# mindazhao/PWStableNet

Hardware: AMD Instinct MI355X
Metric: stabilized frames/sec at 256x256 (netG fp32 + grid_sample), whole job (higher is better)
Workload: dtype f32

## Files before the change

### pwstablenet_amd/csrc/conv_dispatch.hip

```cpp
#include "conv_common.h"

namespace pws {

static inline bool ledger_direct(int bit) { return (exp_mask(EXP_PARITY_LEDGER, 32) & bit) != 0; }

int conv2d_fwd_impl(const pws_conv_args *a, const ConvCtx &cx) {
    PWS_REQUIRE(a != nullptr, "pws_conv2d_fwd: args is NULL");
    PWS_REQUIRE(a->n >= 0 && a->h > 0 && a->w > 0, "pws_conv2d_fwd: bad n/h/w %d/%d/%d", a->n, a->h, a->w);
    PWS_REQUIRE(a->nsrc >= 1 && a->nsrc <= 4, "pws_conv2d_fwd: nsrc %d not in 1..4", a->nsrc);
    PWS_REQUIRE(a->cout > 0 && a->cout % 4 == 0, "pws_conv2d_fwd: cout %d must be a positive multiple of 4", a->cout);
    PWS_REQUIRE(a->out && a->w_packed, "pws_conv2d_fwd: NULL out / w_packed");
    PWS_REQUIRE(a->out_ld >= a->cout, "pws_conv2d_fwd: out_ld %d < cout %d", a->out_ld, a->cout);
    PWS_REQUIRE(a->act >= PWS_ACT_NONE && a->act <= PWS_ACT_RELU, "pws_conv2d_fwd: bad act %d", a->act);
    PWS_REQUIRE(a->ws == nullptr || (reinterpret_cast<size_t>(a->ws) & 15) == 0, "pws_conv2d_fwd: ws must be 16-B aligned");
    if (a->n == 0) return PWS_OK;

    ConvKParams kp{};
    int cin = 0;
    kp.nsrc = a->nsrc;
    const bool nchw = a->src_nchw != 0;
    if (nchw) {
        PWS_REQUIRE(a->kind == PWS_CONV_K5S1 && a->nsrc == 1, "pws_conv2d_fwd: NCHW source only for the k5 first layer");
        PWS_REQUIRE(a->src[0].ptr && a->src[0].channels > 0, "pws_conv2d_fwd: bad NCHW source");
        PWS_REQUIRE(a->src[0].ld >= 0, "pws_conv2d_fwd: NCHW source: ld is the sample stride in floats (0 = dense)");
        kp.src_ptr[0] = a->src[0].ptr, kp.src_c[0] = a->src[0].channels, kp.src_ld[0] = a->src[0].ld;
        cin = a->src[0].channels;
    } else {
        for (int s = 0; s < a->nsrc; ++s) {
            const pws_src &sr = a->src[s];
            PWS_REQUIRE(sr.ptr && sr.channels > 0 && sr.channels % 16 == 0 && sr.ld >= sr.channels && sr.ld % 4 == 0 &&
                            (reinterpret_cast<size_t>(sr.ptr) & 15) == 0,
                        "pws_conv2d_fwd: source %d (channels %d, ld %d) must be 16-B aligned, channels %% 16 == 0, ld %% 4 == 0",
                        s, sr.channels, sr.ld);
            kp.src_ptr[s] = sr.ptr, kp.src_c[s] = sr.channels, kp.src_ld[s] = sr.ld;
            cin += sr.channels;
        }
    }
    kp.cin_pad = (cin + 15) / 16 * 16;
    kp.N = a->n, kp.H = a->h, kp.W = a->w;
    kp.cout = a->cout, kp.w = a->w_packed, kp.bias = a->bias, kp.out_ld = a->out_ld, kp.act = a->act;
    kp.nclasses = 1;
    PWS_REQUIRE((size_t)a->n * a->h * a->w < (1u << 31), "pws_conv2d_fwd: n*h*w too large for 32-bit pixel indices");
    float *ws = static_cast<float *>(a->ws);
    const size_t ws_floats = a->ws_bytes / sizeof(float);
    const bool bf16 = a->math == PWS_MATH_BF16 && a->w_bf16 && !nchw;
    if (a->store == PWS_STORE_BF16) {
        PWS_REQUIRE(bf16, "pws_conv2d_fwd: bf16 storage needs math == PWS_MATH_BF16, w_bf16 and NHWC sources");
        PWS_REQUIRE(a->out_ld % 2 == 0 && a->cout % 2 == 0 && (reinterpret_cast<size_t>(a->out) & 3) == 0,
                    "pws_conv2d_fwd: bf16 storage needs an even cout / out_ld and a 4-byte aligned out");
        for (int s = 0; s < a->nsrc; ++s)
            PWS_REQUIRE(a->src[s].channels % 32 == 0 && a->src[s].ld % 8 == 0,
                        "pws_conv2d_fwd: bf16 storage needs channels %% 32 == 0 and ld %% 8 == 0 (source %d: %d, %d)", s,
                        a->src[s].channels, a->src[s].ld);
        kp.io_bf16 = 1;
        kp.epi16 = a->cout % 8 == 0 && a->out_ld % 8 == 0 && (reinterpret_cast<size_t>(a->out) & 15) == 0;
    }
    kp.w_bf = a->w_bf16, kp.kpad_bf = (kp.cin_pad + 31) / 32 * 32, kp.npad_bf = (a->cout + 63) / 64 * 64;
    if (a->out_sign) {
        PWS_REQUIRE(a->store == PWS_STORE_BF16 && a->cout % 8 == 0 && a->out_sign_ld >= a->cout / 8,
                    "pws_conv2d_fwd: out_sign needs bf16 storage, cout %% 8 == 0 and out_sign_ld >= cout / 8");
        kp.out_sign = a->out_sign, kp.out_sign_ld = a->out_sign_ld;
    }

    const bool fp32_nhwc = !bf16 && !nchw, k5 = a->kind == PWS_CONV_K5S1;
    const bool ringf_on = fp32_nhwc && !k5 && !ledger_direct(8), skinny_on = fp32_nhwc && !k5 && !ledger_direct(16);
    int k2;
    bool wring_on = false, wino_on = false;
    switch (a->kind) {
    case PWS_CONV_K3S1:
    case PWS_CONVT_K3S1: {
        kp.OH = kp.LH = a->h, kp.OW = kp.LW = a->w, k2 = 9;
        wring_on = a->w_wring && fp32_nhwc && !ledger_direct(2);
        const long wblocks = cdiv(a->w, 16) * cdiv(a->h, 16) * a->n * cdiv(a->cout, 64);
        wino_on = a->w_wino && !nchw && a->h >= 16 && a->w >= 16 && wblocks >= 128 && (cin >= 128 || wblocks >= 2048) && !ledger_direct(2);
        break;
    }
    case PWS_CONV_K3S2: kp.OH = kp.LH = (a->h + 2 - 3) / 2 + 1, kp.OW = kp.LW = (a->w + 2 - 3) / 2 + 1, k2 = 9; break;
    case PWS_CONV_K5S1:
        kp.OH = kp.LH = a->h, kp.OW = kp.LW = a->w, k2 = 25;
        ws = nullptr;
        break;
    case PWS_CONVT_K4S2: {
        kp.LH = a->h, kp.LW = a->w, kp.OH = 2 * a->h, kp.OW = 2 * a->w, kp.nclasses = 4, k2 = 4;
        wring_on = a->w_wring && fp32_nhwc && !ledger_direct(4);
        const long wb = cdiv(a->w, 24) * cdiv(a->h, 12) * a->n * cdiv(a->cout, 64) * 4;
        wino_on = a->w_wino && a->h >= 24 && a->w >= 24 && wb >= 256 && !ledger_direct(4);
        break;
    }
    default:
        set_error("pws_conv2d_fwd: kind %d is not a runnable conv kind", a->kind);
        return PWS_EINVAL;
    }
    const double out_pix = (double)a->n * kp.OH * kp.OW, es = a->store == PWS_STORE_BF16 ? 2.0 : 4.0, ws_ = bf16 ? 2.0 : 4.0;
    ProfInfo pi{2.0 * out_pix * a->cout * (double)cin * k2, es * ((double)a->n * a->h * a->w * cin + out_pix * a->cout) + ws_ * (double)k2 * cin * a->cout};
    if (a->kind == PWS_CONVT_K4S2) pi.bytes += ws_ * 12.0 * cin * a->cout;
    int rc = PWS_OK;
    if (bf16 && conv_bf16_fwd(a->kind, kp, kp.cin_pad, a->out, ws, ws_floats, pi, cx, &rc)) return rc;
    if (wring_on && conv_wring(a, pi, cx, &rc)) return rc;
    if (wino_on && conv_wino(a, pi, cx, &rc)) return rc;
    kp.out = a->out;
    if (ringf_on && conv_ringf(a->kind, kp, pi, cx, &rc)) return rc;
    if (skinny_on && conv_skinny(a->kind, kp, a->out, ws, ws_floats, pi, cx, &rc)) return rc;
    if (k5 && nchw && !ledger_direct(1)) {
        if (a->w_wring && conv_first_wino(kp, static_cast<const float *>(a->w_wring), pi, cx, &rc)) return rc;
        if (conv_first(kp, pi, cx, &rc)) return rc;
    }
    conv_mfma(a->kind, false, nchw, kp, kp.cin_pad, a->out, ws, ws_floats, pi, cx, &rc);
    return rc;
}

int conv2d_bwd_data_impl(const pws_conv_bwd_data_args *a, const ConvCtx &cx) {
    PWS_REQUIRE(a != nullptr, "pws_conv2d_bwd_data: args is NULL");
    PWS_REQUIRE(a->n >= 0 && a->h > 0 && a->w > 0 && a->cout > 0 && a->cout % 16 == 0, "pws_conv2d_bwd_data: bad shape");
    PWS_REQUIRE(a->gout && a->w_dgrad && a->gout_ld >= a->cout && a->gout_ld % 4 == 0, "pws_conv2d_bwd_data: bad gout / weights");
    PWS_REQUIRE(a->ndst >= 1 && a->ndst <= 4, "pws_conv2d_bwd_data: ndst %d not in 1..4", a->ndst);
    if (a->n == 0) return PWS_OK;
    ConvKParams kp{};
    int oh = a->h, ow = a->w;
    if (a->kind == PWS_CONV_K3S2) oh = (a->h - 1) / 2 + 1, ow = (a->w - 1) / 2 + 1;
    if (a->kind == PWS_CONVT_K4S2) oh = 2 * a->h, ow = 2 * a->w;
    kp.nsrc = 1, kp.src_ptr[0] = a->gout, kp.src_c[0] = a->cout, kp.src_ld[0] = a->gout_ld;
    kp.N = a->n, kp.H = oh, kp.W = ow;
    kp.OH = a->h, kp.OW = a->w;
    kp.cin_pad = a->cout;
    int cin_f = 0;
    kp.ndst = a->ndst;
    for (int s = 0; s < a->ndst; ++s) {
        const pws_dst &d = a->dst[s];
        PWS_REQUIRE(d.ptr && d.channels > 0 && d.ld >= d.channels, "pws_conv2d_bwd_data: bad destination %d", s);
        kp.dst_ptr[s] = d.ptr, kp.dst_c0[s] = cin_f, kp.dst_c1[s] = cin_f + d.channels, kp.dst_ld[s] = d.ld;
        kp.dst_acc[s] = d.accumulate ? 1 : 0;
        if (d.act_y && d.act != PWS_ACT_NONE) {
            PWS_REQUIRE(a->store == PWS_STORE_BF16 && (d.act == PWS_ACT_LRELU || d.act == PWS_ACT_RELU),
                        "pws_conv2d_bwd_data: the fused act' (dst[%d].act_y) needs bf16 storage and PWS_ACT_LRELU / PWS_ACT_RELU", s);
            PWS_REQUIRE(d.act_y_ld >= d.channels && d.act_y_ld % 2 == 0 && (reinterpret_cast<size_t>(d.act_y) & 3) == 0,
                        "pws_conv2d_bwd_data: bad act_y / act_y_ld of destination %d", s);
            kp.dst_y[s] = d.act_y, kp.dst_y_ld[s] = d.act_y_ld, kp.dst_act[s] = d.act;
            if (d.act_sign) {
                PWS_REQUIRE(d.channels % 8 == 0 && d.act_sign_ld >= d.channels / 8, "pws_conv2d_bwd_data: bad act_sign / act_sign_ld of destination %d", s);
                kp.dst_sign[s] = d.act_sign, kp.dst_sign_ld[s] = d.act_sign_ld;
            }
        }
        cin_f += d.channels;
    }
    PWS_REQUIRE(cin_f % 4 == 0, "pws_conv2d_bwd_data: total destination channels %d must be a multiple of 4", cin_f);
    kp.cout = cin_f, kp.w = a->w_dgrad, kp.bias = nullptr, kp.act = PWS_ACT_NONE, kp.out_ld = cin_f, kp.nclasses = 1;
    PWS_REQUIRE((size_t)a->n * oh * ow < (1u << 31) && (size_t)a->n * a->h * a->w < (1u << 31), "pws_conv2d_bwd_data: too large");
    float *ws = static_cast<float *>(a->ws);
    const size_t ws_floats = a->ws_bytes / sizeof(float);
    ProfInfo pi;
    const double k2 = a->kind == PWS_CONVT_K4S2 ? 4.0 : 9.0;
    pi.flops = 2.0 * a->n * oh * ow * (double)a->cout * cin_f * k2;
    {
        const double es = a->store == PWS_STORE_BF16 ? 2.0 : 4.0, in_pix = (double)a->n * a->h * a->w;
        pi.bytes = es * ((double)a->n * oh * ow * a->cout + in_pix * cin_f);
        for (int s = 0; s < a->ndst; ++s)
            pi.bytes += es * in_pix * a->dst[s].channels * (a->dst[s].accumulate ? 1.0 : 0.0) +
                        (kp.dst_act[s] == PWS_ACT_NONE ? 0.0 : (kp.dst_sign[s] ? in_pix * a->dst[s].channels / 8.0 : es * in_pix * a->dst[s].channels));
    }
    if (a->kind == PWS_CONV_K3S2)
        kp.LH = oh, kp.LW = ow, kp.nclasses = 4;
    else
        kp.LH = a->h, kp.LW = a->w;
    if (a->store == PWS_STORE_BF16) {
        PWS_REQUIRE(a->math == PWS_MATH_BF16 && a->w_dgrad_bf16 && a->cout % 32 == 0 && a->gout_ld % 8 == 0,
                    "pws_conv2d_bwd_data: bf16 storage needs bf16 math, w_dgrad_bf16, cout %% 32 == 0 and gout_ld %% 8 == 0");
        for (int s = 0; s < a->ndst; ++s)
            PWS_REQUIRE(a->dst[s].channels % 2 == 0 && a->dst[s].ld % 2 == 0 && (reinterpret_cast<size_t>(a->dst[s].ptr) & 3) == 0,
                        "pws_conv2d_bwd_data: bf16 storage needs even channels / ld and 4-byte aligned destinations");
        kp.io_bf16 = 1;
        kp.epi16 = 1;
        for (int s = 0; s < a->ndst; ++s)
            if (a->dst[s].channels % 8 || a->dst[s].ld % 8 || (reinterpret_cast<size_t>(a->dst[s].ptr) & 15) ||
                (kp.dst_act[s] != PWS_ACT_NONE && (kp.dst_y_ld[s] % 8 || (reinterpret_cast<size_t>(kp.dst_y[s]) & 15))))
                kp.epi16 = 0;
    }
    int rc = PWS_OK;
    if (a->math == PWS_MATH_BF16 && a->w_dgrad_bf16) {
        kp.w_bf = a->w_dgrad_bf16, kp.kpad_bf = (a->cout + 31) / 32 * 32, kp.npad_bf = (cin_f + 63) / 64 * 64;
        if (conv_bf16_dgrad(a->kind, kp, a->cout, ws, ws_floats, pi, cx, &rc)) return rc;
    }
    if (a->kind != PWS_CONV_K3S1 && a->kind != PWS_CONVT_K3S1 && a->kind != PWS_CONV_K3S2 && a->kind != PWS_CONVT_K4S2) {
        set_error("pws_conv2d_bwd_data: kind %d has no data gradient here", a->kind);
        return PWS_EINVAL;
    }
    conv_mfma(a->kind, true, false, kp, a->cout, nullptr, ws, ws_floats, pi, cx, &rc);
    return rc;
}

}

static pws::ConvCtx run_ctx(pws_stream_t stream) { return pws::ConvCtx{pws::as_stream(stream), pws::device_cus(), true, nullptr}; }
static pws::ConvCtx plan_ctx(int compute_units, pws_conv_choice *out) {
    *out = pws_conv_choice{};
    out->kernel_id = -1;
    return pws::ConvCtx{nullptr, compute_units, false, out};
}

extern "C" int pws_conv2d_fwd(const pws_conv_args *args, pws_stream_t stream) { return pws::conv2d_fwd_impl(args, run_ctx(stream)); }

extern "C" int pws_conv2d_bwd_data(const pws_conv_bwd_data_args *args, pws_stream_t stream) {
    return pws::conv2d_bwd_data_impl(args, run_ctx(stream));
}

extern "C" int pws_conv2d_fwd_plan(const pws_conv_args *args, int compute_units, pws_conv_choice *out) {
    PWS_REQUIRE(out && compute_units > 0, "pws_conv2d_fwd_plan: NULL out / compute_units %d", compute_units);
    return pws::conv2d_fwd_impl(args, plan_ctx(compute_units, out));
}

extern "C" int pws_conv2d_bwd_data_plan(const pws_conv_bwd_data_args *args, int compute_units, pws_conv_choice *out) {
    PWS_REQUIRE(out && compute_units > 0, "pws_conv2d_bwd_data_plan: NULL out / compute_units %d", compute_units);
    return pws::conv2d_bwd_data_impl(args, plan_ctx(compute_units, out));
}
```

### pwstablenet_amd/csrc/conv_mfma.hip

```cpp
#include "conv_common.h"

namespace pws {

template <int KS_, int STRIDE_, int PAD_, int SUBPIX_, int TH_, int TW_, int TN_, int CK_, int WM_, int WN_, int MT_,
          int NT_, bool NCHW_ = false>
struct ConvCfg {
    static constexpr int KS = KS_, STRIDE = STRIDE_, PAD = PAD_, TH = TH_, TW = TW_, TN = TN_, CK = CK_;
    static constexpr int SUBPIX = SUBPIX_;
    static constexpr bool CONVT = SUBPIX_ != 0, NCHW = NCHW_;
    static constexpr int WM = WM_, WN = WN_, MT = MT_, NT = NT_;
    static constexpr int THREADS = 64 * WM * WN;
    static constexpr int BM = TH * TW * TN, BN = 32 * NT * WN;
    static_assert(BM == 32 * MT * WM, "tile pixels must equal the M extent of the wave grid");
    static constexpr int IH = (TH - 1) * STRIDE + KS, IW = (TW - 1) * STRIDE + KS;
    static constexpr int PIX = TN * IH * IW;
    static constexpr int CKP = CK + 1;
    static constexpr int TAPS = KS * KS;
    static constexpr int LDS_IN = (PIX * CKP + 3) / 4 * 4;
    static constexpr int LDS_W = TAPS * CK * BN;
    static constexpr int LDS_BYTES = (LDS_IN + LDS_W) * 4;
    static constexpr int C4 = CK / 4;
    static constexpr int ITEMS_IN = (PIX * C4 + THREADS - 1) / THREADS;
    static constexpr int ITEMS_W = (TAPS * CK * (BN / 4) + THREADS - 1) / THREADS;
    static constexpr int ITEMS_NCHW = (PIX * CK + THREADS - 1) / THREADS;
};

template <class C>
__global__ void __launch_bounds__(C::THREADS, 2) conv_mfma_kernel(const ConvKParams p) {
    extern __shared__ float lds[];
    float *lds_in = lds;
    float *lds_w = lds + C::LDS_IN;

    const int tid = threadIdx.x;
    const int lane = tid & 63, wv = tid >> 6;
    const int l31 = lane & 31, hi = lane >> 5;
    const int wm = wv / C::WN, wn = wv % C::WN;

    unsigned tile;
    int cls, split;
    conv_block_coords(p, C::CONVT, tile, cls, split);
    const int tx_i = tile % p.tiles_x;
    const int ty_i = (tile / p.tiles_x) % p.tiles_y;
    const int tn_i = tile / (p.tiles_x * p.tiles_y);
    const int n0 = tn_i * C::TN, y0 = ty_i * C::TH, x0 = tx_i * C::TW;
    const int co0 = blockIdx.y * C::BN;
    const int py = cls >> 1, px = cls & 1;
    const int pad_y = C::SUBPIX == 1 ? 1 - py : (C::SUBPIX == 2 ? 0 : C::PAD);
    const int pad_x = C::SUBPIX == 1 ? 1 - px : (C::SUBPIX == 2 ? 0 : C::PAD);
    const int iy0 = y0 * C::STRIDE - pad_y, ix0 = x0 * C::STRIDE - pad_x;

    int g_pix[C::ITEMS_IN];
    int l_off[C::ITEMS_IN];
    int g_c4[C::ITEMS_IN];
    unsigned ok_mask = 0;
#pragma unroll
    for (int it = 0; it < C::ITEMS_IN; ++it) {
        const int item = tid + it * C::THREADS;
        const int pix = item / C::C4, c4 = item % C::C4;
        const int lx = pix % C::IW, ly = (pix / C::IW) % C::IH, tn = pix / (C::IW * C::IH);
        const int n = n0 + tn, iy = iy0 + ly, ix = ix0 + lx;
        const bool ok = item < C::PIX * C::C4 && n < p.N && iy >= 0 && iy < p.H && ix >= 0 && ix < p.W;
        g_pix[it] = ok ? (n * p.H + iy) * p.W + ix : 0;
        ok_mask |= ok ? (1u << it) : 0u;
        l_off[it] = item < C::PIX * C::C4 ? pix * C::CKP + c4 * 4 : -1;
        g_c4[it] = c4 * 4;
    }
    static_assert(C::ITEMS_IN <= 32 && C::ITEMS_W <= 32, "mask width");
    int w_off[C::ITEMS_W];
    unsigned w_mask = 0;
#pragma unroll
    for (int it = 0; it < C::ITEMS_W; ++it) {
        const int item = tid + it * C::THREADS;
        const int row = item / (C::BN / 4), q = item % (C::BN / 4);
        const int tap = row / C::CK, c = row % C::CK;
        const bool ok = item < C::TAPS * C::CK * (C::BN / 4) && (co0 + q * 4) < p.cout;
        w_off[it] = ok ? (tap * p.cin_pad + c) * p.cout + co0 + q * 4 : 0;
        w_mask |= ok ? (1u << it) : 0u;
    }
    const float *w_cls = p.w + (size_t)cls * C::TAPS * p.cin_pad * p.cout;
    float4 r_in[C::NCHW ? 1 : C::ITEMS_IN];
    float4 r_w[C::ITEMS_W];
    float r_nchw[C::NCHW ? C::ITEMS_NCHW : 1];

    auto load_chunk = [&](int s, int c0, int wrow) {
        if constexpr (C::NCHW) {
            const int Creal = p.src_c[0];
            const size_t sstride = p.src_ld[0] ? (size_t)p.src_ld[0] : (size_t)Creal * p.H * p.W;
#pragma unroll
            for (int it = 0; it < C::ITEMS_NCHW; ++it) {
                const int item = tid + it * C::THREADS;
                const int c = item / C::PIX, pix = item % C::PIX;
                const int lx = pix % C::IW, ly = (pix / C::IW) % C::IH, tn = pix / (C::IW * C::IH);
                const int n = n0 + tn, iy = iy0 + ly, ix = ix0 + lx;
                const bool ok = item < C::PIX * C::CK && (c0 + c) < Creal && n < p.N && iy >= 0 && iy < p.H && ix >= 0 &&
                                ix < p.W;
                const size_t off = ok ? (size_t)n * sstride + ((size_t)(c0 + c) * p.H + iy) * p.W + ix : 0;
                const float v = p.src_ptr[0][off];
                r_nchw[it] = ok ? v : 0.f;
            }
        } else {
            const float *sp = p.src_ptr[s] + c0;
            const size_t ld = p.src_ld[s];
#pragma unroll
            for (int it = 0; it < C::ITEMS_IN; ++it)
                r_in[it] = *reinterpret_cast<const float4 *>(sp + (size_t)g_pix[it] * ld + g_c4[it]);
        }
        const float *wp = w_cls + (size_t)wrow * p.cout;
#pragma unroll
        for (int it = 0; it < C::ITEMS_W; ++it) r_w[it] = *reinterpret_cast<const float4 *>(wp + w_off[it]);
    };
    auto store_chunk = [&]() {
        if constexpr (C::NCHW) {
#pragma unroll
            for (int it = 0; it < C::ITEMS_NCHW; ++it) {
                const int item = tid + it * C::THREADS;
                const int c = item / C::PIX, pix = item % C::PIX;
                if (item < C::PIX * C::CK) lds_in[pix * C::CKP + c] = r_nchw[it];
            }
        } else {
#pragma unroll
            for (int it = 0; it < C::ITEMS_IN; ++it) {
                if (l_off[it] >= 0) {
                    const bool ok = (ok_mask >> it) & 1u;
                    float *d = lds_in + l_off[it];
                    d[0] = ok ? r_in[it].x : 0.f, d[1] = ok ? r_in[it].y : 0.f, d[2] = ok ? r_in[it].z : 0.f,
                    d[3] = ok ? r_in[it].w : 0.f;
                }
            }
        }
#pragma unroll
        for (int it = 0; it < C::ITEMS_W; ++it) {
            const int item = tid + it * C::THREADS;
            if (item < C::TAPS * C::CK * (C::BN / 4)) {
                const bool ok = (w_mask >> it) & 1u;
                *reinterpret_cast<float4 *>(lds_w + item * 4) =
                    ok ? r_w[it] : make_float4(0.f, 0.f, 0.f, 0.f);
            }
        }
    };

    f32x16 acc[C::MT][C::NT];
#pragma unroll
    for (int mt = 0; mt < C::MT; ++mt)
#pragma unroll
        for (int nt = 0; nt < C::NT; ++nt)
#pragma unroll
            for (int r = 0; r < 16; ++r) acc[mt][nt][r] = 0.f;

    int a_base[C::MT];
#pragma unroll
    for (int mt = 0; mt < C::MT; ++mt) {
        const int m = (wm * C::MT + mt) * 32 + l31;
        const int tx = m % C::TW, ty = (m / C::TW) % C::TH, tn = m / (C::TW * C::TH);
        a_base[mt] = ((tn * C::IH + ty * C::STRIDE) * C::IW + tx * C::STRIDE) * C::CKP + hi;
    }
    const int b_base = hi * C::BN + wn * C::NT * 32 + l31;

    int total_chunks = 0;
    if constexpr (C::NCHW) {
        total_chunks = p.cin_pad / C::CK;
    } else {
        for (int s = 0; s < p.nsrc; ++s) total_chunks += p.src_c[s] / C::CK;
    }
    const int ch_begin = split * p.chunks_per_split;
    const int ch_end = min(total_chunks, ch_begin + p.chunks_per_split);
    int s = 0, c0 = ch_begin * C::CK, wrow = ch_begin * C::CK;
    if constexpr (!C::NCHW) {
        while (s < p.nsrc - 1 && c0 >= p.src_c[s]) c0 -= p.src_c[s], ++s;
    }
    if (ch_begin < ch_end) load_chunk(s, c0, wrow);
    for (int ch = ch_begin; ch < ch_end; ++ch) {
        __syncthreads();
        store_chunk();
        __syncthreads();
        c0 += C::CK, wrow += C::CK;
        if (!C::NCHW && c0 >= p.src_c[s]) ++s, c0 = 0;
        if (ch + 1 < ch_end) load_chunk(s, c0, wrow);

#pragma unroll
        for (int tap = 0; tap < C::TAPS; ++tap) {
            if (C::SUBPIX == 2 && ((!py && tap / C::KS) || (!px && tap % C::KS))) continue;
            const int toff = ((tap / C::KS) * C::IW + (tap % C::KS)) * C::CKP;
#pragma unroll
            for (int kk = 0; kk < C::CK / 2; ++kk) {
                float a[C::MT], b[C::NT];
#pragma unroll
                for (int mt = 0; mt < C::MT; ++mt) a[mt] = lds_in[a_base[mt] + toff + 2 * kk];
#pragma unroll
                for (int nt = 0; nt < C::NT; ++nt) b[nt] = lds_w[b_base + (tap * C::CK + 2 * kk) * C::BN + nt * 32];
#pragma unroll
                for (int mt = 0; mt < C::MT; ++mt)
#pragma unroll
                    for (int nt = 0; nt < C::NT; ++nt)
                        acc[mt][nt] = __builtin_amdgcn_mfma_f32_32x32x2f32(a[mt], b[nt], acc[mt][nt], 0, 0, 0);
            }
        }
    }

    const bool partial = p.ksplit > 1;
    float *part = p.out + (size_t)split * p.split_stride;
#pragma unroll
    for (int nt = 0; nt < C::NT; ++nt) {
        const int co = co0 + (wn * C::NT + nt) * 32 + l31;
        const bool co_ok = co < p.cout;
#pragma unroll
        for (int mt = 0; mt < C::MT; ++mt) {
#pragma unroll
            for (int r = 0; r < 16; ++r) {
                const int m = (wm * C::MT + mt) * 32 + (r & 3) + 8 * (r >> 2) + 4 * hi;
                const int tx = m % C::TW, ty = (m / C::TW) % C::TH, tn = m / (C::TW * C::TH);
                const int n = n0 + tn, y = y0 + ty, x = x0 + tx;
                const int oy = C::CONVT ? 2 * y + py : y, ox = C::CONVT ? 2 * x + px : x;
                if (co_ok && n < p.N && y < p.LH && x < p.LW && oy < p.OH && ox < p.OW) {
                    const size_t pix = (size_t)(n * p.OH + oy) * p.OW + ox;
                    if (partial)
                        part[pix * p.cout + co] = acc[mt][nt][r];
                    else
                        epi_store(p, pix, co, acc[mt][nt][r]);
                }
            }
        }
    }
}

__global__ void __launch_bounds__(256) splitk_reduce_kernel(const ConvKParams p, const float *__restrict__ partial,
                                                            size_t total4) {
    const size_t i = (size_t)blockIdx.x * 256 + threadIdx.x;
    if (i >= total4) return;
    float4 a = reinterpret_cast<const float4 *>(partial)[i];
    for (int s = 1; s < p.ksplit; ++s) {
        const float4 b = reinterpret_cast<const float4 *>(partial + (size_t)s * p.split_stride)[i];
        a.x += b.x, a.y += b.y, a.z += b.z, a.w += b.w;
    }
    const size_t pix = (i * 4) / p.cout;
    const int co = (int)((i * 4) % p.cout);
    if (p.io_bf16) {
        epi_store_pair16(p, pix, co, a.x, a.y), epi_store_pair16(p, pix, co + 2, a.z, a.w);
        return;
    }
    epi_store(p, pix, co, a.x), epi_store(p, pix, co + 1, a.y), epi_store(p, pix, co + 2, a.z), epi_store(p, pix, co + 3, a.w);
}

int launch_splitk_reduce(const ConvKParams &kp, const float *partial, size_t total4, hipStream_t st) {
    hipLaunchKernelGGL(splitk_reduce_kernel, dim3((unsigned)((total4 + 255) / 256)), dim3(256), 0, st, kp, partial, total4);
    return check_launch("splitk_reduce_kernel");
}

template <class C>
static int run_cfg(const ConvKParams &kp, const ConvChoice &c, hipStream_t st) { return launch_planned<&conv_mfma_kernel<C>>(kp, c, st, "conv_mfma_kernel"); }

template <class C, int KID>
static constexpr TileChoice choice() {
    return TileChoice{C::TH, C::TW, C::TN, C::CK, C::BN, KID, {{C::THREADS, C::LDS_BYTES}, {C::THREADS, C::LDS_BYTES}}, &run_cfg<C>};
}

using K3S1_T256 = ConvCfg<3, 1, 1, 0, 16, 16, 1, 16, 4, 1, 2, 2>;
using K3S1_T128 = ConvCfg<3, 1, 1, 0, 8, 16, 1, 16, 4, 1, 1, 2>;
using K3S1_T64 = ConvCfg<3, 1, 1, 0, 8, 8, 1, 16, 2, 2, 1, 1>;
using K3S1_T64N4 = ConvCfg<3, 1, 1, 0, 4, 4, 4, 16, 2, 2, 1, 1>;
using K3S1_T64N16 = ConvCfg<3, 1, 1, 0, 2, 2, 16, 16, 2, 2, 1, 1>;
using K3S2_T256 = ConvCfg<3, 2, 1, 0, 16, 16, 1, 8, 4, 1, 2, 2>;
using K3S2_T128 = ConvCfg<3, 2, 1, 0, 8, 16, 1, 16, 4, 1, 1, 2>;
using K3S2_T64 = ConvCfg<3, 2, 1, 0, 8, 8, 1, 16, 2, 2, 1, 1>;
using K3S2_T64N4 = ConvCfg<3, 2, 1, 0, 4, 4, 4, 16, 2, 2, 1, 1>;
using K3S2_T64N16 = ConvCfg<3, 2, 1, 0, 2, 2, 16, 16, 2, 2, 1, 1>;
using K5S1_T256 = ConvCfg<5, 1, 2, 0, 16, 16, 1, 8, 4, 1, 2, 2>;
using K5S1_T256_NCHW = ConvCfg<5, 1, 2, 0, 16, 16, 1, 8, 4, 1, 2, 2, true>;
using CT4_T256 = ConvCfg<2, 1, 0, 1, 16, 16, 1, 16, 4, 1, 2, 2>;
using CT4_T128 = ConvCfg<2, 1, 0, 1, 8, 16, 1, 16, 4, 1, 1, 2>;
using CT4_T64 = ConvCfg<2, 1, 0, 1, 8, 8, 1, 16, 2, 2, 1, 1>;
using CT4_T64N4 = ConvCfg<2, 1, 0, 1, 4, 4, 4, 16, 2, 2, 1, 1>;
using CT4_T64N16 = ConvCfg<2, 1, 0, 1, 2, 2, 16, 16, 2, 2, 1, 1>;

using K4S2_T256 = ConvCfg<4, 2, 1, 0, 16, 16, 1, 8, 4, 1, 2, 2>;
using K4S2_T128 = ConvCfg<4, 2, 1, 0, 8, 16, 1, 8, 4, 1, 1, 2>;
using K4S2_T64 = ConvCfg<4, 2, 1, 0, 8, 8, 1, 8, 2, 2, 1, 1>;
using K4S2_T64N4 = ConvCfg<4, 2, 1, 0, 4, 4, 4, 8, 2, 2, 1, 1>;
using K4S2_T64N16 = ConvCfg<4, 2, 1, 0, 2, 2, 16, 8, 2, 2, 1, 1>;
using SP3_T256 = ConvCfg<2, 1, 0, 2, 16, 16, 1, 16, 4, 1, 2, 2>;
using SP3_T128 = ConvCfg<2, 1, 0, 2, 8, 16, 1, 16, 4, 1, 1, 2>;
using SP3_T64 = ConvCfg<2, 1, 0, 2, 8, 8, 1, 16, 2, 2, 1, 1>;
using SP3_T64N4 = ConvCfg<2, 1, 0, 2, 4, 4, 4, 16, 2, 2, 1, 1>;
using SP3_T64N16 = ConvCfg<2, 1, 0, 2, 2, 2, 16, 16, 2, 2, 1, 1>;

static const TileChoice kK3S1[] = {choice<K3S1_T256, KID_CONV_K3S1_BIG>(), choice<K3S1_T128, KID_CONV_K3S1_BIG>(),
                                   choice<K3S1_T64, KID_CONV_K3S1_SMALL>(), choice<K3S1_T64N4, KID_CONV_K3S1_SMALL>(),
                                   choice<K3S1_T64N16, KID_CONV_K3S1_SMALL>()};
static const TileChoice kK3S2[] = {choice<K3S2_T256, KID_CONV_K3S2_BIG>(), choice<K3S2_T128, KID_CONV_K3S2_BIG>(),
                                   choice<K3S2_T64, KID_CONV_K3S2_SMALL>(), choice<K3S2_T64N4, KID_CONV_K3S2_SMALL>(),
                                   choice<K3S2_T64N16, KID_CONV_K3S2_SMALL>()};
static const TileChoice kCT4[] = {choice<CT4_T256, KID_CONVT4_BIG>(), choice<CT4_T128, KID_CONVT4_BIG>(),
                                  choice<CT4_T64, KID_CONVT4_SMALL>(), choice<CT4_T64N4, KID_CONVT4_SMALL>(),
                                  choice<CT4_T64N16, KID_CONVT4_SMALL>()};
static const TileChoice kK4S2[] = {choice<K4S2_T256, KID_DGRAD_K4S2>(), choice<K4S2_T128, KID_DGRAD_K4S2>(),
                                   choice<K4S2_T64, KID_DGRAD_K4S2>(), choice<K4S2_T64N4, KID_DGRAD_K4S2>(),
                                   choice<K4S2_T64N16, KID_DGRAD_K4S2>()};
static const TileChoice kSP3[] = {choice<SP3_T256, KID_DGRAD_SP3>(), choice<SP3_T128, KID_DGRAD_SP3>(),
                                  choice<SP3_T64, KID_DGRAD_SP3>(), choice<SP3_T64N4, KID_DGRAD_SP3>(),
                                  choice<SP3_T64N16, KID_DGRAD_SP3>()};
static const TileChoice kK5[] = {choice<K5S1_T256, KID_CONV_K5S1>()};
static const TileChoice kK5N[] = {choice<K5S1_T256_NCHW, KID_CONV_K5S1>()};

bool conv_mfma(int kind, bool dgrad, bool nchw, ConvKParams &kp, int cin_total, float *final_out, float *ws, size_t ws_floats, const ProfInfo &pi,
               const ConvCtx &cx, int *status) {
    const bool s1 = kind == PWS_CONV_K3S1 || kind == PWS_CONVT_K3S1, k5 = kind == PWS_CONV_K5S1;
    const TileChoice *cands = s1 ? kK3S1 : k5 ? (nchw ? kK5N : kK5) : kind == PWS_CONV_K3S2 ? (dgrad ? kSP3 : kK3S2) : (dgrad ? kK4S2 : kCT4);
    const int ncand = k5 ? 1 : 5;
    ConvChoice c;
    const TileChoice *t = plan_tiles(cands, ncand, kp, cin_total, final_out, ws, ws_floats, kFillBlocks, 0, &c);
    return conv_accept(cx, c, pi, status, [&] { return run_tiles(*t, c, kp, final_out, ws, cx.stream); });
}

}
```

### pwstablenet_amd/csrc/experiments.h

```cpp
#pragma once

namespace pws {

extern int g_experiment;

enum Exp : int {
    EXP_GS_BWD_GENERAL = 2,
    EXP_U8_CVT_SHIFT = 4,
    EXP_GS_ROWWIN = 5,
    EXP_NO_SIGN_BITS = 12,
    EXP_NETG_PER_STAGE = 15,
    EXP_RING_OFF = 20,
    EXP_RING_SMALL = 21,
    EXP_RINGF_OFF = 22,
    EXP_RINGF_8X32 = 23,
    EXP_RINGF_16X32 = 24,
    EXP_FIRST_MFMA = 25,
    EXP_FIRST_NO_WINO = 26,
    EXP_RINGF_32CH = 27,
    EXP_FIRST_SMALL = 29,
    EXP_WINO5_SMALL = 30,
    EXP_HEAD_V1 = 35,
    EXP_GS_U8_LANE_WINDOWS = 49,
    EXP_WRING_OFF = 50,
    EXP_WRING_FORCE = 58,
    EXP_WRING_MODE2 = 59,
    EXP_SKINNY_OFF = 70,
    EXP_SKINNY16_OFF = 71,
    EXP_SKINNY16_4096 = 72,
    EXP_SKINNY_SKIP = 73,
    EXP_WGRAD_RING_OFF = 80,
    EXP_WGRAD_RING_FORCE = 81,
    EXP_HEAD_VALU = 90,
    EXP_HEAD_BWD_VALU = 91,
    EXP_HEAD_ONE_TILE = 92,
    EXP_DEEP_TILE_ALWAYS = 96,
    EXP_SHAPE_GENERAL = 97,
    EXP_TL1_TILED = 98,
    EXP_RING_8WAVE = 105,
    EXP_SMOOTH_ONE_PIXEL = 110,
    EXP_NO_PACK_ONE_PASS = 120,
    EXP_RING_UNIT256 = 186,
    EXP_RING_UNIT128 = 187,
    EXP_WGRAD_NO_MERGE = 188,
    EXP_WGRAD_MIN_TILES = 190,
    EXP_FIRST_ABLATE = 1100,
    EXP_FIRST_CLOCK = 1200,
    EXP_WINO5_ABLATE = 1300,
    EXP_WGRAD_WIDE_ABLATE = 1400,
    EXP_RING_ABLATE = 1500,
    EXP_WINO_ABLATE = 1600,
    EXP_BF16_PROBE = 2100,
    EXP_RINGF_VARIANT = 2200,
    EXP_PARITY_LEDGER = 3000,
    EXP_WRING_ABLATE = 4000,
};

inline bool exp_is(Exp e) { return g_experiment == e; }
inline bool exp_in(Exp base, int n) { return g_experiment >= base && g_experiment < base + n; }
inline int exp_mask(Exp base, int n) { return exp_in(base, n) ? g_experiment - base : 0; }

}
```

### pwstablenet_amd/hipabi.py

```python
import contextlib
import ctypes
import os

_HERE = os.path.dirname(os.path.abspath(__file__))
LIB_PATH = os.environ.get("PWS_LIB_PATH") or os.path.join(_HERE, "libpwstable_hip.so")

c_f32p = ctypes.c_void_p
c_stream = ctypes.c_void_p

ACT_NONE, ACT_LRELU, ACT_RELU = 0, 1, 2
OPT_TWO_QUEUES = 1
OPT_MATH, MATH_FP32, MATH_BF16 = 2, 0, 1
OPT_STORE, STORE_FP32, STORE_BF16 = 3, 0, 1
ABI_VERSION = 5
NETG_DETERMINISTIC = 1
NETG_PRUNE_DEAD = 2
OPT_EXPERIMENT = 100


class Exp:
    GS_BWD_GENERAL = 2
    U8_CVT_SHIFT = 4
    GS_ROWWIN = 5
    NO_SIGN_BITS = 12
    NETG_PER_STAGE = 15
    RING_OFF = 20
    RING_SMALL = 21
    RINGF_OFF = 22
    RINGF_8X32 = 23
    RINGF_16X32 = 24
    FIRST_MFMA = 25
    FIRST_NO_WINO = 26
    RINGF_32CH = 27
    FIRST_SMALL = 29
    WINO5_SMALL = 30
    HEAD_V1 = 35
    GS_U8_LANE_WINDOWS = 49
    WRING_OFF = 50
    WRING_FORCE = 58
    WRING_MODE2 = 59
    SKINNY_OFF = 70
    SKINNY16_OFF = 71
    SKINNY16_4096 = 72
    SKINNY_SKIP = 73
    WGRAD_RING_OFF = 80
    WGRAD_RING_FORCE = 81
    HEAD_VALU = 90
    HEAD_BWD_VALU = 91
    HEAD_ONE_TILE = 92
    DEEP_TILE_ALWAYS = 96
    SHAPE_GENERAL = 97
    TL1_TILED = 98
    RING_8WAVE = 105
    SMOOTH_ONE_PIXEL = 110
    NO_PACK_ONE_PASS = 120
    RING_UNIT256 = 186
    RING_UNIT128 = 187
    WGRAD_NO_MERGE = 188
    WGRAD_MIN_TILES = 190
    FIRST_ABLATE = 1100
    FIRST_CLOCK = 1200
    WINO5_ABLATE = 1300
    WGRAD_WIDE_ABLATE = 1400
    RING_ABLATE = 1500
    WINO_ABLATE = 1600
    BF16_PROBE = 2100
    RINGF_VARIANT = 2200
    PARITY_LEDGER = 3000
    WRING_ABLATE = 4000
OBJ_SLOTS = 64
CONV_K3S1, CONV_K3S2, CONV_K5S1, CONVT_K3S1, CONVT_K4S2, CONV_K2S1P0, CONV_K1, CONV_K3S1_OUT = range(8)


class PwsSrc(ctypes.Structure):
    _fields_ = [("ptr", ctypes.c_void_p), ("channels", ctypes.c_int), ("ld", ctypes.c_int)]


class PwsConvArgs(ctypes.Structure):
    _fields_ = [("kind", ctypes.c_int), ("n", ctypes.c_int), ("h", ctypes.c_int), ("w", ctypes.c_int),
                ("nsrc", ctypes.c_int), ("src", PwsSrc * 4), ("src_nchw", ctypes.c_int), ("cout", ctypes.c_int),
                ("w_packed", ctypes.c_void_p), ("bias", ctypes.c_void_p), ("act", ctypes.c_int),
                ("out", ctypes.c_void_p), ("out_ld", ctypes.c_int), ("w_wino", ctypes.c_void_p), ("ws", ctypes.c_void_p),
                ("ws_bytes", ctypes.c_size_t), ("math", ctypes.c_int), ("w_bf16", ctypes.c_void_p), ("store", ctypes.c_int),
                ("w_wring", ctypes.c_void_p), ("out_sign", ctypes.c_void_p), ("out_sign_ld", ctypes.c_int)]


class PwsDst(ctypes.Structure):
    _fields_ = [("ptr", ctypes.c_void_p), ("channels", ctypes.c_int), ("ld", ctypes.c_int), ("accumulate", ctypes.c_int),
                ("act_y", ctypes.c_void_p), ("act_y_ld", ctypes.c_int), ("act", ctypes.c_int),
                ("act_sign", ctypes.c_void_p), ("act_sign_ld", ctypes.c_int)]


class PwsConvBwdDataArgs(ctypes.Structure):
    _fields_ = [("kind", ctypes.c_int), ("n", ctypes.c_int), ("h", ctypes.c_int), ("w", ctypes.c_int), ("cout", ctypes.c_int),
                ("gout", ctypes.c_void_p), ("gout_ld", ctypes.c_int), ("w_dgrad", ctypes.c_void_p), ("ndst", ctypes.c_int),
                ("dst", PwsDst * 4), ("ws", ctypes.c_void_p), ("ws_bytes", ctypes.c_size_t), ("math", ctypes.c_int),
                ("w_dgrad_bf16", ctypes.c_void_p), ("store", ctypes.c_int)]


class PwsConvBwdWeightArgs(ctypes.Structure):
    _fields_ = [("kind", ctypes.c_int), ("n", ctypes.c_int), ("h", ctypes.c_int), ("w", ctypes.c_int), ("nsrc", ctypes.c_int),
                ("src", PwsSrc * 4), ("src_nchw", ctypes.c_int), ("cout", ctypes.c_int), ("gout", ctypes.c_void_p),
                ("gout_ld", ctypes.c_int), ("dw_packed", ctypes.c_void_p), ("math", ctypes.c_int), ("store", ctypes.c_int),
                ("dbias", ctypes.c_void_p), ("deterministic", ctypes.c_int), ("src2_ptr", ctypes.c_void_p * 4), ("gout2", ctypes.c_void_p)]


class PwsNetgOpts(ctypes.Structure):
    _fields_ = [("math", ctypes.c_int), ("store", ctypes.c_int), ("two_queues", ctypes.c_int), ("flags", ctypes.c_int),
                ("x_sample_stride", ctypes.c_size_t)]


class PwsConvChoice(ctypes.Structure):
    _fields_ = [("kernel_id", ctypes.c_int), ("variant", ctypes.c_int * 4), ("grid", ctypes.c_uint * 3), ("threads", ctypes.c_int),
                ("lds_bytes", ctypes.c_int), ("ksplit", ctypes.c_int), ("follow", ctypes.c_int), ("tag", ctypes.c_int)]

    def as_dict(self, L):
        return {"tag": self.tag, "kernel": L.pws_prof_kernel_name(self.kernel_id).decode(), "variant": list(self.variant),
                "grid": list(self.grid), "threads": self.threads, "lds_bytes": self.lds_bytes, "ksplit": self.ksplit, "follow": self.follow}


class PwsProfRecord(ctypes.Structure):
    _fields_ = [("kernel_id", ctypes.c_int), ("tag", ctypes.c_int), ("flops", ctypes.c_double),
                ("bytes", ctypes.c_double), ("ms", ctypes.c_float)]


_I, _S, _P = ctypes.c_int, ctypes.c_size_t, ctypes.c_void_p
_F = ctypes.c_float
_D = ctypes.c_double
SIGNATURES = {
    "pws_version": (_I, []),
    "pws_last_error": (ctypes.c_char_p, []),
    "pws_set_option": (_I, [_I, _I]),
    "pws_get_option": (_I, [_I]),
    "pws_packed_bf16_floats": (_S, [_I, _I, _I]),
    "pws_pack_weight_bf16": (_I, [_P, _P, _I, _I, _I, _P]),
    "pws_nchw_to_nhwc_pad": (_I, [_P, _P, _I, _I, _I, _I, _I, _P]),
    "pws_nchw_to_nhwc_pad_s": (_I, [_P, _P, _I, _I, _I, _I, _I, _I, _P]),
    "pws_cvt_bf16_to_f32": (_I, [_P, _P, _S, _P]),
    "pws_cvt_f32_to_bf16": (_I, [_P, _P, _S, _I, _P]),
    "pws_device_info": (_I, [ctypes.POINTER(_I), ctypes.POINTER(_I)]),
    "pws_packed_weight_floats": (_S, [_I, _I, _I]),
    "pws_pack_conv_weight": (_I, [_P, _P, _I, _I, _I, _P]),
    "pws_packed_wino_floats": (_S, [_I, _I]),
    "pws_pack_conv_weight_wino": (_I, [_P, _P, _I, _I, _P]),
    "pws_packed_wring_floats": (_S, [_I, _I, _I]),
    "pws_pack_conv_weight_wring": (_I, [_P, _P, _I, _I, _I, _P]),
    "pws_packed_wino_ct4_floats": (_S, [_I, _I]),
    "pws_pack_conv_weight_wino_ct4": (_I, [_P, _P, _I, _I, _P]),
    "pws_conv2d_fwd": (_I, [ctypes.POINTER(PwsConvArgs), _P]),
    "pws_act_bwd_bias": (_I, [_P, _P, _S, _I, _I, _P, _P]),
    "pws_act_bwd_bias_s": (_I, [_P, _P, _S, _I, _I, _P, _I, _P, _S, _P]),
    "pws_act_bwd_bias_ws_bytes": (_S, [_I]),
    "pws_packed_dgrad_floats": (_S, [_I, _I, _I]),
    "pws_pack_conv_weight_dgrad": (_I, [_P, _P, _I, _I, _I, _P]),
    "pws_conv2d_bwd_data": (_I, [ctypes.POINTER(PwsConvBwdDataArgs), _P]),
    "pws_conv2d_fwd_plan": (_I, [ctypes.POINTER(PwsConvArgs), _I, ctypes.POINTER(PwsConvChoice)]),
    "pws_conv2d_bwd_data_plan": (_I, [ctypes.POINTER(PwsConvBwdDataArgs), _I, ctypes.POINTER(PwsConvChoice)]),
    "pws_netg_forward_plan": (_I, [_I, _I, _I, _I, ctypes.POINTER(PwsNetgOpts), _I, ctypes.POINTER(PwsConvChoice), _I]),
    "pws_conv2d_bwd_weight": (_I, [ctypes.POINTER(PwsConvBwdWeightArgs), _P]),
    "pws_unpack_conv_weight": (_I, [_P, _P, _I, _I, _I, _P]),
    "pws_theta_head_fwd_save": (_I, [_P, _I, _I, _I, _P, _P, _P, _P, _P, _P, _P, _P]),
    "pws_theta_head_bwd": (_I, [_P, _I, _I, _I, _P, _P, _P, _P, _P, _P, _P, _P, _P, _P, _I, _P, _P]),
    "pws_field_head_bwd": (_I, [_P, _I, _I, _I, _I, _I, _P, _P, _P, _P, _I, _P, _I, _I, _P, _P, _P, _P, _P]),
    "pws_field_head_bwd_s": (_I, [_P, _I, _I, _I, _I, _I, _P, _P, _P, _P, _I, _P, _I, _I, _P, _P, _P, _P, _I, _P]),
    "pws_field_head_bwd_act": (_I, [_P, _I, _I, _I, _I, _I, _P, _P, _P, _P, _I, _P, _I, _I, _P, _P, _P, _P, _I, _I, _P]),
    "pws_netg_packed_dgrad_floats": (_S, [_I, _I]),
    "pws_netg_pack_weights_dgrad": (_I, [ctypes.POINTER(_P), _P, _I, _I, _P]),
    "pws_netg_train_workspace_bytes": (_S, [_I, _I, _I]),
    "pws_netg_backward": (_I, [_P, _P, _P, _I, _I, _I, _I, _P, _S, _P, _P, _P, _P, _P, _P]),
    "pws_netg_backward_part": (_I, [_P, _P, _P, _I, _I, _I, _I, _P, _S, _P, _P, _P, _P, _P, _I, _I, _P, _P]),
    "pws_netg_bn_floats": (_S, [_I, _I]),
    "pws_netg_train_workspace_bytes_bn": (_S, [_I, _I, _I]),
    "pws_netg_forward_bn": (_I, [_P, _P, _P, _F, _F, _P, _I, _I, _I, _I, _P, _S, _P, _P, _P, _P]),
    "pws_netg_backward_bn": (_I, [_P, _P, _P, _F, _P, _I, _I, _I, _I, _P, _S, _P, _P, _P, _P, _P, _P, _P]),
    "pws_netg_forward_bn_opts": (_I, [_P, _P, _P, _F, _F, _P, _I, _I, _I, _I, _P, _S, _P, _P, _P, ctypes.POINTER(PwsNetgOpts), _P]),
    "pws_netg_backward_bn_opts": (_I, [_P, _P, _P, _F, _P, _I, _I, _I, _I, _P, _S, _P, _P, _P, _P, _P, _P, ctypes.POINTER(PwsNetgOpts), _P]),
    "pws_netg_unpack_grads": (_I, [_P, ctypes.POINTER(_P), _I, _I, _P]),
    "pws_theta_head_ws_floats": (_S, [_I, _I, _I]),
    "pws_theta_head_fwd": (_I, [_P, _I, _I, _I, _P, _P, _P, _P, _P, _P, _P]),
    "pws_field_head_fwd": (_I, [_P, _I, _I, _I, _I, _I, _P, _P, _P, _I, _P, _P, _P]),
    "pws_field_head_fwd_s": (_I, [_P, _I, _I, _I, _I, _I, _P, _P, _P, _I, _P, _P, _I, _P]),
    "pws_affine_grid": (_I, [_P, _P, _I, _I, _I, _I, _P]),
    "pws_grid_sample_fwd": (_I, [_P, _P, _P, _I, _I, _I, _I, _I, _I, _I, _P]),
    "pws_grid_sample_bwd": (_I, [_P, _P, _P, _P, _P, _I, _I, _I, _I, _I, _I, _I, _P]),
    "pws_upsample_bilinear_ac": (_I, [_P, _P, _I, _I, _I, _I, _I, _I, _P]),
    "pws_upsample_bilinear_ac_bwd": (_I, [_P, _P, _I, _I, _I, _I, _I, _I, _P]),
    "pws_affine_grid_bwd": (_I, [_P, _P, _I, _I, _I, _I, _P]),
    "pws_upsample_grid_sample_fwd": (_I, [_P, _P, _P, _I, _I, _I, _I, _I, _I, _I, _P]),
    "pws_upsample_grid_sample_u8": (_I, [_P, _P, _P, _I, _I, _I, _I, _I, _I, _I, _P]),
    "pws_adam_step": (_I, [_P, _P, _P, _P, _S, _F, _F, _F, _F, _I, _P]),
    "pws_adam_step_multi": (_I, [_P, _P, _P, _P, _P, _I, _F, _F, _F, _F, _I, _P]),
    "pws_netg_packed_floats": (_S, [_I, _I]),
    "pws_netg_pack_weights": (_I, [ctypes.POINTER(_P), _P, _I, _I, _P]),
    "pws_netg_pack_weights_for": (_I, [ctypes.POINTER(_P), _P, _I, _I, _I, _P]),
    "pws_netg_pack_weights_train": (_I, [ctypes.POINTER(_P), _P, _P, _I, _I, _I, _P]),
    "pws_netg_workspace_bytes": (_S, [_I, _I, _I, _I]),
    "pws_netg_forward": (_I, [_P, _P, _I, _I, _I, _I, _I, _P, _S, _P, _P, _P, _P]),
    "pws_netg_forward_opts": (_I, [_P, _P, _I, _I, _I, _I, _I, _P, _S, _P, _P, _P, ctypes.POINTER(PwsNetgOpts), _P]),
    "pws_netg_backward_opts": (_I, [_P, _P, _P, _I, _I, _I, _I, _P, _S, _P, _P, _P, _P, _P, _I, _I, _P, ctypes.POINTER(PwsNetgOpts), _P]),
    "pws_netg_backward_lists": (_I, [_P, _P, _P, _I, _I, _I, _I, _P, _S, _P, _P, ctypes.POINTER(_P), ctypes.POINTER(_P), _P, _I, _I, _P,
                                     ctypes.POINTER(PwsNetgOpts), _P]),
    "pws_netg_grad_floats": (_S, [_I, _I]),
    "pws_netg_grad_layout": (_I, [_I, _I, ctypes.POINTER(_S), ctypes.POINTER(_S)]),
    "pws_netg_backward_plan": (_I, [_I, _I, _I, ctypes.POINTER(ctypes.c_ubyte)]),
    "pws_u8_normalize": (_I, [_P, _S, _P, _S, _I, _S, _P]),
    "pws_warp_norm_fwd": (_I, [_P, _S, _P, _P, _P, _S, _P, _I, _I, _I, _P]),
    "pws_warp_norm_bwd": (_I, [_P, _S, _P, _P, _S, _F, _P, _P, _P, _I, _I, _I, _I, _P]),
    "pws_temporal_l1_fwd": (_I, [_P, _P, _P, _P, _I, _I, _I, _P]),
    "pws_temporal_l1_bwd": (_I, [_P, _P, _P, _F, _P, _P, _P, _I, _I, _I, _P]),
    "pws_temporal_l1_bwd_det": (_I, [_P, _P, _P, _F, _P, _P, _P, _P, _I, _I, _I, _P]),
    "pws_feature_loss_fwd": (_I, [_P, _P, _P, _I, _I, _I, _I, _P]),
    "pws_feature_loss_bwd": (_I, [_P, _P, _F, _P, _P, _I, _I, _I, _I, _P]),
    "pws_feature_loss_bwd_det": (_I, [_P, _P, _F, _P, _P, _I, _I, _I, _I, _P]),
    "pws_field_smoothness": (_I, [_P, _P, _P, _I, _I, _I, _P]),
    "pws_shape_loss_fwd": (_I, [_P, _P, _I, _I, _I, _P]),
    "pws_shape_loss_bwd": (_I, [_P, ctypes.c_double, _P, _P, _I, _I, _I, _P]),
    "pws_objective_finalize": (_I, [_P, _I, _P, _I, _P, _P]),
    "pws_maxpool2x2_fwd": (_I, [_P, _P, _I, _I, _I, _I, _P]),
    "pws_maxpool2x2_bwd": (_I, [_P, _P, _P, _I, _I, _I, _I, _P]),
    "pws_maxpool2x2_fwd_s": (_I, [_P, _P, _I, _I, _I, _I, _I, _P]),
    "pws_maxpool2x2_bwd_s": (_I, [_P, _P, _P, _I, _I, _I, _I, _I, _I, _P]),
# ... 154 lines not shown
```

Before: 2024.

## Software-pipeline LDS reads ahead of MFMA in single-tile conv kernel and batch split-K reduce

```diff
diff --git a/pwstablenet_amd/csrc/conv_dispatch.hip b/pwstablenet_amd/csrc/conv_dispatch.hip
--- a/pwstablenet_amd/csrc/conv_dispatch.hip
+++ b/pwstablenet_amd/csrc/conv_dispatch.hip
@@ -63,7 +63,8 @@
     }
 
     const bool fp32_nhwc = !bf16 && !nchw, k5 = a->kind == PWS_CONV_K5S1;
-    const bool ringf_on = fp32_nhwc && !k5 && !ledger_direct(8), skinny_on = fp32_nhwc && !k5 && !ledger_direct(16);
+    const bool ringf_on = fp32_nhwc && !k5 && !ledger_direct(8);
+    const bool skinny_on = fp32_nhwc && !k5 && !ledger_direct(16) && exp_mask(EXP_DEEP_PARENT, 2) != 1;
     int k2;
     bool wring_on = false, wino_on = false;
     switch (a->kind) {
diff --git a/pwstablenet_amd/csrc/conv_mfma.hip b/pwstablenet_amd/csrc/conv_mfma.hip
--- a/pwstablenet_amd/csrc/conv_mfma.hip
+++ b/pwstablenet_amd/csrc/conv_mfma.hip
@@ -23,10 +23,13 @@
     static constexpr int ITEMS_IN = (PIX * C4 + THREADS - 1) / THREADS;
     static constexpr int ITEMS_W = (TAPS * CK * (BN / 4) + THREADS - 1) / THREADS;
     static constexpr int ITEMS_NCHW = (PIX * CK + THREADS - 1) / THREADS;
+    static constexpr bool PIPE = MT == 1 && NT == 1 && SUBPIX != 2 && KS != 4 && !NCHW;
 };
 
-template <class C>
-__global__ void __launch_bounds__(C::THREADS, 2) conv_mfma_kernel(const ConvKParams p) {
+constexpr int CONV_V_NO_MFMA = 1, CONV_V_NO_READS = 2, CONV_V_NO_STAGE = 4, CONV_V_NO_STORE = 8, CONV_V_PARENT = 16;
+
+template <class C, int V>
+__device__ __forceinline__ void conv_mfma_body(const ConvKParams &p) {
     extern __shared__ float lds[];
     float *lds_in = lds;
     float *lds_w = lds + C::LDS_IN;
@@ -168,31 +171,59 @@
     if constexpr (!C::NCHW) {
         while (s < p.nsrc - 1 && c0 >= p.src_c[s]) c0 -= p.src_c[s], ++s;
     }
+    constexpr bool PIPE = C::PIPE && !(V & CONV_V_PARENT);
+    constexpr int STEPS = C::TAPS * (C::CK / 2);
     if (ch_begin < ch_end) load_chunk(s, c0, wrow);
     for (int ch = ch_begin; ch < ch_end; ++ch) {
         __syncthreads();
-        store_chunk();
+        if (!(V & CONV_V_NO_STAGE) || ch == ch_begin) store_chunk();
         __syncthreads();
         c0 += C::CK, wrow += C::CK;
         if (!C::NCHW && c0 >= p.src_c[s]) ++s, c0 = 0;
-        if (ch + 1 < ch_end) load_chunk(s, c0, wrow);
-
-#pragma unroll
-        for (int tap = 0; tap < C::TAPS; ++tap) {
-            if (C::SUBPIX == 2 && ((!py && tap / C::KS) || (!px && tap % C::KS))) continue;
-            const int toff = ((tap / C::KS) * C::IW + (tap % C::KS)) * C::CKP;
-#pragma unroll
-            for (int kk = 0; kk < C::CK / 2; ++kk) {
-                float a[C::MT], b[C::NT];
-#pragma unroll
-                for (int mt = 0; mt < C::MT; ++mt) a[mt] = lds_in[a_base[mt] + toff + 2 * kk];
-#pragma unroll
-                for (int nt = 0; nt < C::NT; ++nt) b[nt] = lds_w[b_base + (tap * C::CK + 2 * kk) * C::BN + nt * 32];
-#pragma unroll
-                for (int mt = 0; mt < C::MT; ++mt)
-#pragma unroll
-                    for (int nt = 0; nt < C::NT; ++nt)
-                        acc[mt][nt] = __builtin_amdgcn_mfma_f32_32x32x2f32(a[mt], b[nt], acc[mt][nt], 0, 0, 0);
+        if (ch + 1 < ch_end && !(V & CONV_V_NO_STAGE)) load_chunk(s, c0, wrow);
+
+        if constexpr (PIPE) {
+            constexpr int PF = 2;
+            float ra[PF + 1], rb[PF + 1];
+            auto rd = [&](int i, float &a, float &b) {
+                const int tap = i / (C::CK / 2), kk = i % (C::CK / 2);
+                if constexpr (V & CONV_V_NO_READS) {
+                    a = __builtin_bit_cast(float, 0x3f800000 + lane), b = __builtin_bit_cast(float, 0x3f800000 + tid);
+                } else {
+                    a = lds_in[a_base[0] + ((tap / C::KS) * C::IW + (tap % C::KS)) * C::CKP + 2 * kk];
+                    b = lds_w[b_base + (tap * C::CK + 2 * kk) * C::BN];
+                }
+            };
+#pragma unroll
+            for (int i = 0; i < PF; ++i) rd(i, ra[i], rb[i]);
+#pragma unroll
+            for (int i = 0; i < STEPS; ++i) {
+                if (i + PF < STEPS) rd(i + PF, ra[(i + PF) % (PF + 1)], rb[(i + PF) % (PF + 1)]);
+                __builtin_amdgcn_sched_barrier(0);
+                if constexpr (V & CONV_V_NO_MFMA)
+                    asm volatile("" ::"v"(ra[i % (PF + 1)]), "v"(rb[i % (PF + 1)]));
+                else
+                    acc[0][0] = __builtin_amdgcn_mfma_f32_32x32x2f32(ra[i % (PF + 1)], rb[i % (PF + 1)], acc[0][0], 0, 0, 0);
+                __builtin_amdgcn_sched_barrier(0);
+            }
+        } else {
+#pragma unroll
+            for (int tap = 0; tap < C::TAPS; ++tap) {
+                if (C::SUBPIX == 2 && ((!py && tap / C::KS) || (!px && tap % C::KS))) continue;
+                const int toff = ((tap / C::KS) * C::IW + (tap % C::KS)) * C::CKP;
+#pragma unroll
+                for (int kk = 0; kk < C::CK / 2; ++kk) {
+                    float a[C::MT], b[C::NT];
+#pragma unroll
+                    for (int mt = 0; mt < C::MT; ++mt) a[mt] = lds_in[a_base[mt] + toff + 2 * kk];
+#pragma unroll
+                    for (int nt = 0; nt < C::NT; ++nt) b[nt] = lds_w[b_base + (tap * C::CK + 2 * kk) * C::BN + nt * 32];
+#pragma unroll
+                    for (int mt = 0; mt < C::MT; ++mt)
+#pragma unroll
+                        for (int nt = 0; nt < C::NT; ++nt)
+                            acc[mt][nt] = __builtin_amdgcn_mfma_f32_32x32x2f32(a[mt], b[nt], acc[mt][nt], 0, 0, 0);
+                }
             }
         }
     }
@@ -211,7 +242,7 @@
                 const int tx = m % C::TW, ty = (m / C::TW) % C::TH, tn = m / (C::TW * C::TH);
                 const int n = n0 + tn, y = y0 + ty, x = x0 + tx;
                 const int oy = C::CONVT ? 2 * y + py : y, ox = C::CONVT ? 2 * x + px : x;
-                if (co_ok && n < p.N && y < p.LH && x < p.LW && oy < p.OH && ox < p.OW) {
+                if ((V & CONV_V_NO_STORE) ? p.N < 0 : co_ok && n < p.N && y < p.LH && x < p.LW && oy < p.OH && ox < p.OW) {
                     const size_t pix = (size_t)(n * p.OH + oy) * p.OW + ox;
                     if (partial)
                         part[pix * p.cout + co] = acc[mt][nt][r];
@@ -223,8 +254,58 @@
     }
 }
 
+template <class C>
+__global__ void __launch_bounds__(C::THREADS, 2) conv_mfma_kernel(const ConvKParams p) { conv_mfma_body<C, 0>(p); }
+template <class C, int V>
+__global__ void __launch_bounds__(C::THREADS, 2) conv_mfma_variant_kernel(const ConvKParams p) { conv_mfma_body<C, V>(p); }
+
+__device__ __forceinline__ void splitk_finish(const ConvKParams &p, size_t i, const float4 &a) {
+    const size_t pix = (i * 4) / p.cout;
+    const int co = (int)((i * 4) % p.cout);
+    if (p.io_bf16) {
+        epi_store_pair16(p, pix, co, a.x, a.y), epi_store_pair16(p, pix, co + 2, a.z, a.w);
+        return;
+    }
+    epi_store(p, pix, co, a.x), epi_store(p, pix, co + 1, a.y), epi_store(p, pix, co + 2, a.z), epi_store(p, pix, co + 3, a.w);
+}
+
+template <int N>
+__device__ __forceinline__ void splitk_add_group(float4 &a, const float *q, size_t stride) {
+    float4 b[N];
+#pragma unroll
+    for (int j = 0; j < N; ++j) b[j] = *reinterpret_cast<const float4 *>(q + (size_t)j * stride);
+#pragma unroll
+    for (int j = 0; j < N; ++j) a.x += b[j].x, a.y += b[j].y, a.z += b[j].z, a.w += b[j].w;
+}
+
+constexpr int kReduceGroup = 8;
+
 __global__ void __launch_bounds__(256) splitk_reduce_kernel(const ConvKParams p, const float *__restrict__ partial,
                                                             size_t total4) {
+    const size_t i = (size_t)blockIdx.x * 256 + threadIdx.x;
+    if (i >= total4) return;
+    const float *q = partial + i * 4;
+    const size_t stride = p.split_stride;
+    float4 a = *reinterpret_cast<const float4 *>(q);
+    int s = 1;
+    for (; s + kReduceGroup <= p.ksplit; s += kReduceGroup) splitk_add_group<kReduceGroup>(a, q + (size_t)s * stride, stride);
+    q += (size_t)s * stride;
+    switch (p.ksplit - s) {
+    case 1: splitk_add_group<1>(a, q, stride); break;
+    case 2: splitk_add_group<2>(a, q, stride); break;
+    case 3: splitk_add_group<3>(a, q, stride); break;
+    case 4: splitk_add_group<4>(a, q, stride); break;
+    case 5: splitk_add_group<5>(a, q, stride); break;
+    case 6: splitk_add_group<6>(a, q, stride); break;
+    case 7: splitk_add_group<7>(a, q, stride); break;
+    default: break;
+    }
+    static_assert(kReduceGroup == 8, "the tail switch lists the cases 1 .. kReduceGroup - 1");
+    splitk_finish(p, i, a);
+}
+
+__global__ void __launch_bounds__(256) splitk_reduce_parent_kernel(const ConvKParams p, const float *__restrict__ partial,
+                                                                   size_t total4) {
     const size_t i = (size_t)blockIdx.x * 256 + threadIdx.x;
     if (i >= total4) return;
     float4 a = reinterpret_cast<const float4 *>(partial)[i];
@@ -232,22 +313,44 @@
         const float4 b = reinterpret_cast<const float4 *>(partial + (size_t)s * p.split_stride)[i];
         a.x += b.x, a.y += b.y, a.z += b.z, a.w += b.w;
     }
-    const size_t pix = (i * 4) / p.cout;
-    const int co = (int)((i * 4) % p.cout);
-    if (p.io_bf16) {
-        epi_store_pair16(p, pix, co, a.x, a.y), epi_store_pair16(p, pix, co + 2, a.z, a.w);
-        return;
-    }
-    epi_store(p, pix, co, a.x), epi_store(p, pix, co + 1, a.y), epi_store(p, pix, co + 2, a.z), epi_store(p, pix, co + 3, a.w);
+    splitk_finish(p, i, a);
 }
 
 int launch_splitk_reduce(const ConvKParams &kp, const float *partial, size_t total4, hipStream_t st) {
-    hipLaunchKernelGGL(splitk_reduce_kernel, dim3((unsigned)((total4 + 255) / 256)), dim3(256), 0, st, kp, partial, total4);
+    const dim3 grid((unsigned)((total4 + 255) / 256));
+    if (exp_in(EXP_DEEP_PARENT, 2))
+        hipLaunchKernelGGL(splitk_reduce_parent_kernel, grid, dim3(256), 0, st, kp, partial, total4);
+    else
+        hipLaunchKernelGGL(splitk_reduce_kernel, grid, dim3(256), 0, st, kp, partial, total4);
     return check_launch("splitk_reduce_kernel");
 }
 
+template <class C, int V>
+static int run_variant(const ConvKParams &kp, const ConvChoice &c, hipStream_t st) {
+    return launch_planned<&conv_mfma_variant_kernel<C, V>>(kp, c, st, "conv_mfma_kernel");
+}
+
 template <class C>
-static int run_cfg(const ConvKParams &kp, const ConvChoice &c, hipStream_t st) { return launch_planned<&conv_mfma_kernel<C>>(kp, c, st, "conv_mfma_kernel"); }
+static int run_cfg(const ConvKParams &kp, const ConvChoice &c, hipStream_t st) {
+    if constexpr (C::PIPE) {
+        if (exp_in(EXP_DEEP_PARENT, 2)) return run_variant<C, CONV_V_PARENT>(kp, c, st);
+        if (const int mask = exp_mask(EXP_MFMA_ABLATE, 16)) {
+            if constexpr (C::TN == 1) {
+                switch (mask) {
+                case 1: return run_variant<C, 1>(kp, c, st);
+                case 2: return run_variant<C, 2>(kp, c, st);
+                case 4: return run_variant<C, 4>(kp, c, st);
+                case 8: return run_variant<C, 8>(kp, c, st);
+                case 15: return run_variant<C, 15>(kp, c, st);
+                default: break;
+                }
+            }
+            set_error("conv_mfma_kernel: ablation mask %d is not instantiated for this tile", mask);
+            return PWS_EINVAL;
+        }
+    }
+    return launch_planned<&conv_mfma_kernel<C>>(kp, c, st, "conv_mfma_kernel");
+}
 
 template <class C, int KID>
 static constexpr TileChoice choice() {
diff --git a/pwstablenet_amd/csrc/experiments.h b/pwstablenet_amd/csrc/experiments.h
--- a/pwstablenet_amd/csrc/experiments.h
+++ b/pwstablenet_amd/csrc/experiments.h
@@ -53,6 +53,8 @@
     EXP_BF16_PROBE = 2100,
     EXP_RINGF_VARIANT = 2200,
     EXP_PARITY_LEDGER = 3000,
+    EXP_DEEP_PARENT = 3100,
+    EXP_MFMA_ABLATE = 3200,
     EXP_WRING_ABLATE = 4000,
 };
 
diff --git a/pwstablenet_amd/hipabi.py b/pwstablenet_amd/hipabi.py
--- a/pwstablenet_amd/hipabi.py
+++ b/pwstablenet_amd/hipabi.py
@@ -67,6 +67,8 @@
     BF16_PROBE = 2100
     RINGF_VARIANT = 2200
     PARITY_LEDGER = 3000
+    DEEP_PARENT = 3100
+    MFMA_ABLATE = 3200
     WRING_ABLATE = 4000
 OBJ_SLOTS = 64
 CONV_K3S1, CONV_K3S2, CONV_K5S1, CONVT_K3S1, CONVT_K4S2, CONV_K2S1P0, CONV_K1, CONV_K3S1_OUT = range(8)
```

Result: no change. 2039, median of 6 (+0.7%).
